# NilFoundation/crypto3-zk

Hardware: AMD Instinct MI355X
Metric: MSM Mpoints/sec, BLS12-381 G1 Pippenger, 2^20 points per GPU (higher is better)
Workload: dtype u32; 1 GPU; BLS12-381 G1 Pippenger MSM, ONE MSM of 1 x 2^20 random points/scalars, bases resident; points_per_gpu=1048576, parallelism=point-range partition x1 + one all-gather of the 144-B partial sums

## Files before the change

crypto3-zk_amd/csrc/curve.hpp:

```cpp
#pragma once
#include "fu.hpp"
#include "glv.hpp"

namespace zkhip {

template <class F>
struct Affine {
    F x, y;
    ZK_HD bool is_inf() const { return FieldOps<F>::is_exact_zero(x) && FieldOps<F>::is_exact_zero(y); }
    ZK_HD static Affine infinity() { return {F::zero(), F::zero()}; }
};

template <class F>
struct XYZZ {
    F X, Y, ZZ, ZZZ;
    ZK_HD bool is_inf() const { return FieldOps<F>::is_exact_zero(ZZ); }
    ZK_HD static XYZZ infinity() { return {F::zero(), F::zero(), F::zero(), F::zero()}; }
    ZK_HD static XYZZ from_affine(const Affine<F> &p) {
        if (p.is_inf()) return infinity();
        return {p.x, p.y, F::one(), F::one()};
    }
};

template <class F>
struct Jacobian {
    F X, Y, Z;
};

template <class F>
ZK_HD XYZZ<F> xyzz_dbl_affine(const Affine<F> &p) {
    typedef FieldOps<F> O;
    if (p.is_inf()) return XYZZ<F>::infinity();
    F U = O::add(p.y, p.y);
    F V = O::sqr(U);
    F W = O::mul(U, V);
    F S = O::mul(p.x, V);
    F xx = O::sqr(p.x);
    F M = O::add(O::add(xx, xx), xx);
    F X3 = O::template sub<O::K1>(O::sqr(M), O::add(S, S));
    F Y3 = O::template mul_sub<O::K2>(M, O::template sub<O::K2>(S, X3), W, p.y);
    return {X3, Y3, V, W};
}

template <class F>
ZK_HD XYZZ<F> xyzz_dbl(const XYZZ<F> &a) {
    typedef FieldOps<F> O;
    if (a.is_inf()) return XYZZ<F>::infinity();
    F U = O::add(a.Y, a.Y);
    F V = O::sqr(U);
    F W = O::mul(U, V);
    F S = O::mul(a.X, V);
    F xx = O::sqr(a.X);
    F M = O::add(O::add(xx, xx), xx);
    F X3 = O::template sub<O::K1>(O::sqr(M), O::add(S, S));
    F Y3 = O::template mul_sub<O::K2>(M, O::template sub<O::K2>(S, X3), W, a.Y);
    return {X3, Y3, O::mul(V, a.ZZ), O::mul(W, a.ZZZ)};
}

template <class F>
ZK_HD XYZZ<F> xyzz_madd(const XYZZ<F> &a, const Affine<F> &p_in, bool negate = false) {
    typedef FieldOps<F> O;
    if (p_in.is_inf()) return a;
    Affine<F> p = p_in;
    if (negate) p.y = O::template sub<O::K1>(F::zero(), p.y);
    if (a.is_inf()) return {p.x, p.y, F::one(), F::one()};
    F U2 = O::mul(p.x, a.ZZ);
    F S2 = O::mul(p.y, a.ZZZ);
    F Pd = O::template sub<O::K2>(U2, a.X);
    F R = O::template sub<O::K2>(S2, a.Y);
    F PP = O::sqr(Pd);
    if (O::is_zero_product(PP)) {
        if (O::is_zero(R)) return xyzz_dbl_affine(p);
        return XYZZ<F>::infinity();
    }
    F PPP = O::mul(Pd, PP);
    F Q = O::mul(a.X, PP);
    F X3 = O::template sub<O::K1>(O::sqr(R), O::add(PPP, O::add(Q, Q)));
    F Y3 = O::template mul_sub<O::K2>(R, O::template sub<O::K2>(Q, X3), a.Y, PPP);
    return {X3, Y3, O::mul(a.ZZ, PP), O::mul(a.ZZZ, PPP)};
}

template <class F>
ZK_HD XYZZ<F> xyzz_add(const XYZZ<F> &a, const XYZZ<F> &b) {
    typedef FieldOps<F> O;
    if (a.is_inf()) return b;
    if (b.is_inf()) return a;
    F U1 = O::mul(a.X, b.ZZ);
    F U2 = O::mul(b.X, a.ZZ);
    F S1 = O::mul(a.Y, b.ZZZ);
    F S2 = O::mul(b.Y, a.ZZZ);
    F Pd = O::template sub<O::K1>(U2, U1);
    F R = O::template sub<O::K1>(S2, S1);
    F PP = O::sqr(Pd);
    if (O::is_zero_product(PP)) {
        if (O::is_zero(R)) return xyzz_dbl(a);
        return XYZZ<F>::infinity();
    }
    F PPP = O::mul(Pd, PP);
    F Q = O::mul(U1, PP);
    F X3 = O::template sub<O::K1>(O::sqr(R), O::add(PPP, O::add(Q, Q)));
    F Y3 = O::template mul_sub<O::K1>(R, O::template sub<O::K2>(Q, X3), S1, PPP);
    return {X3, Y3, O::mul(O::mul(a.ZZ, b.ZZ), PP), O::mul(O::mul(a.ZZZ, b.ZZZ), PPP)};
}

template <class F>
ZK_HD XYZZ<F> xyzz_mul_small(const XYZZ<F> &a, uint32_t k) {
    XYZZ<F> r = XYZZ<F>::infinity();
    if (k == 0 || a.is_inf()) return r;
    int top = 31;
    while (!((k >> top) & 1)) --top;
    if (top == 0) return a;
    const XYZZ<F> a2 = xyzz_dbl(a), a3 = xyzz_add(a2, a);
    for (int i = top >> 1; i >= 0; --i) {
        if (!r.is_inf()) r = xyzz_dbl(xyzz_dbl(r));
        const uint32_t d = (k >> (2 * i)) & 3u;
        if (d != 0) r = xyzz_add(r, d == 1 ? a : (d == 2 ? a2 : a3));
    }
    return r;
}

template <class F>
ZK_HD Jacobian<F> xyzz_to_jacobian(const XYZZ<F> &a) {
    typedef FieldOps<F> O;
    if (a.is_inf()) return {F::one(), F::one(), F::zero()};
    F z2 = O::sqr(a.ZZ);
    F z3 = O::sqr(a.ZZZ);
    return {O::mul(a.X, O::sqr(z2)), O::mul(a.Y, O::sqr(z3)), O::mul(a.ZZ, a.ZZZ)};
}

template <class F>
ZK_HD XYZZ<F> xyzz_from_jacobian(const Jacobian<F> &j) {
    typedef FieldOps<F> O;
    if (O::is_zero(j.Z)) return XYZZ<F>::infinity();
    F zz = O::sqr(j.Z);
    return {j.X, j.Y, zz, O::mul(zz, j.Z)};
}

template <class F>
ZK_HD Affine<F> xyzz_to_affine(const XYZZ<F> &a) {
    typedef FieldOps<F> O;
    if (a.is_inf()) return Affine<F>::infinity();
    F i = O::inv(O::mul(a.ZZ, a.ZZZ));
    return {O::mul(a.X, O::mul(i, a.ZZZ)), O::mul(a.Y, O::mul(i, a.ZZ))};
}

template <class F>
ZK_HD Affine<F> affine_load(const uint32_t *p) {
    typedef FieldOps<F> O;
    return {O::load(p), O::load(p + O::WORDS)};
}
template <class F>
ZK_HD void affine_store(uint32_t *p, const Affine<F> &a) {
    typedef FieldOps<F> O;
    O::store(p, a.x);
    O::store(p + O::WORDS, a.y);
}
template <class F>
ZK_HD XYZZ<F> xyzz_load(const uint32_t *p) {
    typedef FieldOps<F> O;
    constexpr int W = O::WORDS;
    return {O::load(p), O::load(p + W), O::load(p + 2 * W), O::load(p + 3 * W)};
}
template <class F>
ZK_HD void xyzz_store(uint32_t *p, const XYZZ<F> &a) {
    typedef FieldOps<F> O;
    constexpr int W = O::WORDS;
    O::store(p, a.X);
    O::store(p + W, a.Y);
    O::store(p + 2 * W, a.ZZ);
    O::store(p + 3 * W, a.ZZZ);
}

template <class F>
ZK_HD void xyzz_store_canonical_jacobian(uint32_t *dst, const XYZZ<F> &p) {
    constexpr int CW = FieldOps<F>::CANON_WORDS;
    Jacobian<F> j = xyzz_to_jacobian(p);
    FieldOps<F>::to_canonical(dst, j.X);
    FieldOps<F>::to_canonical(dst + CW, j.Y);
    FieldOps<F>::to_canonical(dst + 2 * CW, j.Z);
}

template <class F>
ZK_HD void xyzz_park(uint32_t *pt, uint32_t *pre_slot, const XYZZ<F> &q, F &pre) {
    typedef FieldOps<F> O;
    xyzz_store<F>(pt, q);
    if (!q.is_inf()) pre = O::mul(pre, O::mul(q.ZZ, q.ZZZ));
    O::store(pre_slot, pre);
}
template <class F, class Pt, class Pre, class Out>
ZK_HD void xyzz_parked_to_affine(const F &pre_all, uint32_t cnt, Pt pt, Pre pre, Out out) {
    typedef FieldOps<F> O;
    F inv = O::inv(pre_all);
    for (uint32_t k = cnt; k-- > 0;) {
        XYZZ<F> q = xyzz_load<F>(pt(k));
        if (q.is_inf()) {
            affine_store<F>(out(k), Affine<F>::infinity());
            continue;
        }
        F before = k > 0 ? O::load(pre(k - 1)) : F::one();
        F dinv = O::mul(inv, before);
        inv = O::mul(inv, O::mul(q.ZZ, q.ZZZ));
        Affine<F> a = {O::mul(q.X, O::mul(dinv, q.ZZZ)), O::mul(q.Y, O::mul(dinv, q.ZZ))};
        affine_store<F>(out(k), a);
    }
}
constexpr uint32_t AFFINE_MAX_CHUNK = 8;
inline uint32_t affine_chunk(size_t points) {
    uint32_t chunk = 1;
    while (chunk < AFFINE_MAX_CHUNK && (points + chunk - 1) / chunk > 16384) chunk <<= 1;
    return chunk;
}

template <int CURVE, int GROUP>
struct CurveTraits;
template <>
struct CurveTraits<CURVE_BLS12_381, GROUP_G1> {
    typedef bls_fqu F;
};
template <>
struct CurveTraits<CURVE_BLS12_381, GROUP_G2> {
    typedef bls_fqu2 F;
};
template <>
struct CurveTraits<CURVE_BN254, GROUP_G1> {
    typedef bn_fqu F;
};
template <>
struct CurveTraits<CURVE_BN254, GROUP_G2> {
    typedef bn_fqu2 F;
};
template <>
struct CurveTraits<CURVE_PALLAS, GROUP_G1> {
    typedef pallas_fqu F;
};
template <>
// ... 27 lines not shown
```

crypto3-zk_amd/csrc/msm_bucket_acc.hpp:

```cpp
#pragma once
#include "curve.hpp"
#include "fu2_pair.hpp"

namespace zkhip {

template <class F>
struct LimbView;
template <class U>
struct LimbView<Fu<U>> {
    static constexpr int N = U::L;
    ZK_D static uint32_t get(const Fu<U> &x, int i) { return x.v[i]; }
    ZK_D static void set(Fu<U> &x, int i, uint32_t v) { x.v[i] = v; }
};
template <class U>
struct LimbView<Fu2h<U>> {
    static constexpr int N = U::L;
    ZK_D static uint32_t get(const Fu2h<U> &x, int i) { return x.v.v[i]; }
    ZK_D static void set(Fu2h<U> &x, int i, uint32_t v) { x.v.v[i] = v; }
};

template <class F, int NT>
struct LdsAcc {
    typedef LimbView<F> V;
    static constexpr int Q = (V::N + 3) / 4;
    static constexpr size_t BYTES = (size_t)3 * Q * NT * 16;
    uint4 *base;
    uint32_t t;
    ZK_D F get(int coord) const {
        uint32_t w[4 * Q];
#pragma unroll
        for (int q = 0; q < Q; ++q) {
            uint4 v = base[(coord * Q + q) * NT + t];
            w[4 * q] = v.x, w[4 * q + 1] = v.y, w[4 * q + 2] = v.z, w[4 * q + 3] = v.w;
        }
        F r;
#pragma unroll
        for (int i = 0; i < V::N; ++i) V::set(r, i, w[i]);
        return r;
    }
    ZK_D void put(int coord, const F &x) const {
#pragma unroll
        for (int q = 0; q < Q; ++q) {
            uint4 v;
            v.x = 4 * q + 0 < V::N ? V::get(x, 4 * q + 0) : 0u;
            v.y = 4 * q + 1 < V::N ? V::get(x, 4 * q + 1) : 0u;
            v.z = 4 * q + 2 < V::N ? V::get(x, 4 * q + 2) : 0u;
            v.w = 4 * q + 3 < V::N ? V::get(x, 4 * q + 3) : 0u;
            base[(coord * Q + q) * NT + t] = v;
        }
    }
};

template <class F, int NT, int WAVES, int LPB = 1>
__global__ __launch_bounds__(NT, WAVES) void msm_bucket_acc_lds(const uint32_t *__restrict__ bases, const uint32_t *__restrict__ offs,
                                                           const uint32_t *__restrict__ idx, uint32_t nbuckets, uint32_t large,
                                                           const uint32_t *__restrict__ order, uint32_t *__restrict__ buckets) {
    typedef FieldOps<F> O;
    constexpr int NL = O::WORDS;
    extern __shared__ __attribute__((aligned(16))) uint4 acc_lds[];
    const uint32_t tid = threadIdx.x, slot = (blockIdx.x * NT + tid) / LPB;
    if (slot >= nbuckets) return;
    const uint32_t g = order[slot];
    const uint32_t lo = offs[g], hi = offs[g + 1];
    if (hi - lo > large) return;
    LdsAcc<F, NT> A = {acc_lds, tid};
    enum { CX = 0, CY = 1, CZZ = 2 };
    F ZZZ = F::zero();
    bool inf = true;
    for (uint32_t k = lo; k < hi; ++k) {
        const uint32_t e = idx[k];
        Affine<F> p = affine_load<F>(bases + (size_t)(e & 0x7FFFFFFFu) * (2 * NL));
        if (p.is_inf()) continue;
        if (e >> 31) p.y = O::template sub<O::K1>(F::zero(), p.y);
        if (inf) {
            A.put(CX, p.x);
            A.put(CY, p.y);
            A.put(CZZ, F::one());
            ZZZ = F::one();
            inf = false;
            continue;
        }
        F Pd = O::template sub<O::K2>(O::mul(p.x, A.get(CZZ)), A.get(CX));
        F R = O::template sub<O::K2>(O::mul(p.y, ZZZ), A.get(CY));
        F PP = O::sqr(Pd);
        if (O::is_zero_product(PP)) {
            if (O::is_zero(R)) {
                XYZZ<F> d = xyzz_dbl_affine(p);
                A.put(CX, d.X);
                A.put(CY, d.Y);
                A.put(CZZ, d.ZZ);
                ZZZ = d.ZZZ;
            } else {
                inf = true;
            }
            continue;
        }
        F PPP = O::mul(Pd, PP);
        F Q = O::mul(A.get(CX), PP);
        F X3 = O::template sub<O::K1>(O::sqr(R), O::add(PPP, O::add(Q, Q)));
        F Y3 = O::template mul_sub<O::K2>(R, O::template sub<O::K2>(Q, X3), A.get(CY), PPP);
        A.put(CX, X3);
        A.put(CY, Y3);
        A.put(CZZ, O::mul(A.get(CZZ), PP));
        ZZZ = O::mul(ZZZ, PPP);
    }
    XYZZ<F> out = XYZZ<F>::infinity();
    if (!inf) out = {A.get(CX), A.get(CY), A.get(CZZ), ZZZ};
    xyzz_store<F>(buckets + (size_t)g * (4 * NL), out);
}

}
```

crypto3-zk_amd/csrc/msm_core.hpp:

```cpp
#pragma once
#include <algorithm>
#include <string>
#include <type_traits>
#include <vector>

#ifndef ZK_NOINLINE_MUL2
#define ZK_NOINLINE_MUL2 1
#endif
#include "ctx.hpp"
#include "curve.hpp"
#include "msm_entries.hpp"
#include "msm_ops.hpp"
#include "msm_recode.hpp"
#include "msm_bucket_acc.hpp"
#include "fu_pair.hpp"
#include "fu_quad.hpp"
#include "fu_wide.hpp"

namespace {

using namespace zkhip;

#ifndef MSM_G1_THREADS
#define MSM_G1_THREADS 64
// ... 42 lines not shown
    const uint32_t nlarge = plan[1], t = threadIdx.x / LPB;
    for (uint32_t j = blockIdx.x; j < nlarge; j += gridDim.x) {
        const uint32_t g = large[3 * j], first = large[3 * j + 1], nt = large[3 * j + 2];
        XYZZ<F> acc = XYZZ<F>::infinity();
        for (uint32_t k = t; k < nt; k += 64 / LPB) acc = xyzz_add(acc, xyzz_load<F>(partials + (size_t)(first + k) * (4 * NL)));
        if (nt > 1) {
            xyzz_store<F>(lds + (size_t)t * (4 * NL), acc);
            __syncthreads();
            for (uint32_t d = 32 / LPB; d >= 1; d >>= 1) {
                if (t < d && t + d < nt) {
                    acc = xyzz_add(xyzz_load<F>(lds + (size_t)t * (4 * NL)), xyzz_load<F>(lds + (size_t)(t + d) * (4 * NL)));
                    xyzz_store<F>(lds + (size_t)t * (4 * NL), acc);
                }
                __syncthreads();
            }
        }
        if (t == 0) xyzz_store<F>(buckets + (size_t)g * (4 * NL), acc);
        __syncthreads();
    }
}

template <class F, int LPB>
__global__ __launch_bounds__(256) void msm_bucket_merge(uint32_t *__restrict__ buckets, uint32_t B, uint32_t q, uint32_t cur) {
    constexpr int NL = FieldOps<F>::WORDS;
    uint32_t g = (blockIdx.x * blockDim.x + threadIdx.x) / LPB;
    if (g >= q * B) return;
    const uint32_t s = g / B;
    uint32_t *dst = buckets + (size_t)g * (4 * NL);
    XYZZ<F> acc = xyzz_load<F>(dst);
    for (uint32_t k = 1; k < 4; ++k)
        if (s + k * q < cur) acc = xyzz_add(acc, xyzz_load<F>(buckets + ((size_t)g + (size_t)k * q * B) * (4 * NL)));
    xyzz_store<F>(dst, acc);
}

constexpr int MSM_TAIL_THREADS = 256;

template <class F>
ZK_D XYZZ<F> block_tree_sum(uint32_t *lds, XYZZ<F> acc, uint32_t t, uint32_t nthreads) {
    constexpr int NL = FieldOps<F>::WORDS;
    xyzz_store<F>(lds + (size_t)t * (4 * NL), acc);
    __syncthreads();
    for (uint32_t d = nthreads / 2; d >= 1; d >>= 1) {
        if (t < d) {
            acc = xyzz_add(xyzz_load<F>(lds + (size_t)t * (4 * NL)), xyzz_load<F>(lds + (size_t)(t + d) * (4 * NL)));
            xyzz_store<F>(lds + (size_t)t * (4 * NL), acc);
        }
        __syncthreads();
    }
    return acc;
}

template <class F, int LPB>
#ifndef ZK_TAIL_WAVES
#define ZK_TAIL_WAVES 2
#endif
__global__ __launch_bounds__(MSM_TAIL_THREADS, ZK_TAIL_WAVES) void msm_bucket_red(const uint32_t *__restrict__ buckets, uint32_t B, uint32_t L, uint32_t nseg,
                                                                   uint32_t nblk, uint32_t *__restrict__ partial) {
    constexpr int NL = FieldOps<F>::WORDS;
    extern __shared__ __attribute__((aligned(16))) uint32_t lds[];
    constexpr uint32_t SLOTS = MSM_TAIL_THREADS / LPB;
    const uint32_t t = threadIdx.x / LPB, w = blockIdx.x / nblk, seg = (blockIdx.x % nblk) * SLOTS + t;
    XYZZ<F> sum = XYZZ<F>::infinity();
    if (seg < nseg) {
        const uint32_t *base = buckets + ((size_t)w * B + (size_t)seg * L) * (4 * NL);
        if (L == 1) {
            sum = xyzz_mul_small(xyzz_load<F>(base), seg + 1);
        } else {
            XYZZ<F> run = XYZZ<F>::infinity();
            for (int b = (int)L - 1; b >= 0; --b) {
                run = xyzz_add(run, xyzz_load<F>(base + (size_t)b * (4 * NL)));
                sum = xyzz_add(sum, run);
            }
            if (seg != 0) sum = xyzz_add(sum, xyzz_mul_small(run, seg * L));
        }
    }
    sum = block_tree_sum<F>(lds, sum, t, SLOTS);
    if (t == 0) xyzz_store<F>(partial + (size_t)blockIdx.x * (4 * NL), sum);
}

template <class F, int LPB>
__global__ __launch_bounds__(256) void msm_window_sum(const uint32_t *__restrict__ partial, uint32_t nblk, uint32_t *__restrict__ winsum) {
    constexpr int NL = FieldOps<F>::WORDS;
    extern __shared__ __attribute__((aligned(16))) uint32_t lds[];
    const uint32_t w = blockIdx.x, t = threadIdx.x / LPB, slots = blockDim.x / LPB;
    XYZZ<F> acc = XYZZ<F>::infinity();
    for (uint32_t j = t; j < nblk; j += slots) acc = xyzz_add(acc, xyzz_load<F>(partial + ((size_t)w * nblk + j) * (4 * NL)));
    if (nblk > 1) acc = block_tree_sum<F>(lds, acc, t, slots);
    if (t == 0) xyzz_store<F>(winsum + (size_t)w * (4 * NL), acc);
}
inline uint32_t msm_window_threads(uint32_t nblk, int lanes_per_point) { return (size_t)nblk * lanes_per_point > 128 ? 256u : 64u; }

struct MsmFold {
    uint32_t B, C, R, log_c;
    uint32_t run;
    uint32_t m_row, m_col;
};
inline MsmFold msm_fold_geom(const zkhip_ctx *ctx, uint32_t B) {
    MsmFold g;
    int lb = 0;
    while ((1u << lb) < B) ++lb;
    g.B = B;
    g.log_c = (uint32_t)((lb + 1) / 2);
    g.C = 1u << g.log_c;
    g.R = B >> g.log_c;
    g.run = ctx->opt_msm_fold_run > 0 ? (uint32_t)ctx->opt_msm_fold_run : (B >= (1u << 18) ? 8u : 4u);
    g.run = std::max(1u, std::min(g.run, g.R));
    g.m_row = g.C / g.run;
    g.m_col = g.R / g.run;
    return g;
}

template <class FA, int LA, class FT, int LT>
__global__ __launch_bounds__(MSM_TAIL_THREADS, ZK_TAIL_WAVES) void msm_fold(const uint32_t *__restrict__ buckets, MsmFold g, uint32_t *__restrict__ level2) {
    constexpr int NL = FieldOps<FA>::WORDS;
    constexpr uint32_t SA = MSM_TAIL_THREADS / LA, ST = MSM_TAIL_THREADS / LT, PW = 4 * NL;
    extern __shared__ __attribute__((aligned(16))) uint32_t lds[];
    const uint32_t half_wgs = g.B / (SA * g.run);
    const uint32_t w = blockIdx.x / (2 * half_wgs), k = blockIdx.x % (2 * half_wgs);
    const bool col = k >= half_wgs;
    const uint32_t wg = col ? k - half_wgs : k, s = threadIdx.x / LA;
    const uint32_t m = col ? g.m_col : g.m_row, G = SA / m;
    uint32_t first, stride, slot;
    if (!col) {
        first = (wg * G + s / m) * g.C + s % m;
        stride = m;
        slot = s;
    } else {
        const uint32_t j = s / G, ll = s % G;
        first = j * g.C + wg * G + ll;
        stride = m * g.C;
        slot = ll * m + j;
    }
    {
        const uint32_t *src = buckets + ((size_t)w * g.B + first) * PW;
        XYZZ<FA> acc = xyzz_load<FA>(src);
        for (uint32_t i = 1; i < g.run; ++i) acc = xyzz_add(acc, xyzz_load<FA>(src + (size_t)i * stride * PW));
        xyzz_store<FA>(lds + (size_t)slot * PW, acc);
    }
    __syncthreads();
    const uint32_t t = threadIdx.x / LT;
    for (uint32_t half = m / 2; half >= 1; half >>= 1) {
        const uint32_t adds = G * half;
        for (uint32_t idx = t; idx < adds; idx += ST) {
            uint32_t *p = lds + (size_t)((idx / half) * m + idx % half) * PW;
            xyzz_store<FT>(p, xyzz_add(xyzz_load<FT>(p), xyzz_load<FT>(p + (size_t)half * PW)));
        }
        __syncthreads();
    }
    for (uint32_t i = t; i < G; i += ST) {
        const uint32_t o = wg * G + i;
        if (col || o != 0)
            xyzz_store<FT>(level2 + (((size_t)2 * w + (col ? 0 : 1)) * g.C + (col ? o : o - 1)) * PW, xyzz_load<FT>(lds + (size_t)i * m * PW));
    }
}

template <class F, int LPB>
__global__ __launch_bounds__(64) void msm_final_fold(const uint32_t *__restrict__ winsum, uint32_t count, uint32_t shift, uint32_t *const *__restrict__ outs,
                                                     uint32_t *__restrict__ out) {
    constexpr int NL = FieldOps<F>::WORDS;
    if (blockIdx.x >= count || threadIdx.x >= LPB) return;
    XYZZ<F> acc = xyzz_load<F>(winsum + ((size_t)2 * blockIdx.x + 1) * (4 * NL));
    if (!acc.is_inf())
        for (uint32_t i = 0; i < shift; ++i) acc = xyzz_dbl(acc);
    acc = xyzz_add(acc, xyzz_load<F>(winsum + (size_t)2 * blockIdx.x * (4 * NL)));
    xyzz_store_canonical_jacobian<F>(outs ? outs[blockIdx.x] : out, acc);
}

constexpr uint32_t MSM_WIDE_WAVES = 8;

template <class U>
ZK_D XYZZ<FuW<U>> wide_tree_sum(uint32_t *lds, XYZZ<FuW<U>> acc, uint32_t w, uint32_t nw) {
    constexpr uint32_t PW = 4 * U::SL;
    wide_store<U>(lds + w * PW, acc);
    __syncthreads();
    for (uint32_t d = nw / 2; d >= 1; d >>= 1) {
        if (w < d) {
            acc = xyzz_add(wide_load<U>(lds + w * PW), wide_load<U>(lds + (w + d) * PW));
            wide_store<U>(lds + w * PW, acc);
        }
        __syncthreads();
    }
    return acc;
}

template <class U>
__global__ __launch_bounds__(MSM_WIDE_WAVES * 64) void msm_wide_weigh(const uint32_t *__restrict__ points, uint32_t C, uint32_t *__restrict__ partial) {
    constexpr uint32_t PW = 4 * U::SL;
    __shared__ uint32_t lds[MSM_WIDE_WAVES * PW];
    const uint32_t w = threadIdx.x >> 6, i = blockIdx.x * MSM_WIDE_WAVES + w;
    XYZZ<FuW<U>> acc = xyzz_mul_small(wide_load<U>(points + (size_t)i * PW), (i & (C - 1)) + 1);
    acc = wide_tree_sum<U>(lds, acc, w, MSM_WIDE_WAVES);
    if (w == 0) wide_store<U>(partial + (size_t)blockIdx.x * PW, acc);
}

template <class U>
__global__ __launch_bounds__(MSM_WIDE_WAVES * 64) void msm_wide_tree(const uint32_t *__restrict__ in, uint32_t *__restrict__ out) {
    constexpr uint32_t PW = 4 * U::SL;
    __shared__ uint32_t lds[MSM_WIDE_WAVES * PW];
    const uint32_t w = threadIdx.x >> 6;
    const uint32_t *src = in + ((size_t)blockIdx.x * 2 * MSM_WIDE_WAVES + w) * PW;
    XYZZ<FuW<U>> acc = xyzz_add(wide_load<U>(src), wide_load<U>(src + (size_t)MSM_WIDE_WAVES * PW));
    acc = wide_tree_sum<U>(lds, acc, w, MSM_WIDE_WAVES);
    if (w == 0) wide_store<U>(out + (size_t)blockIdx.x * PW, acc);
}

template <class U>
__global__ __launch_bounds__(MSM_WIDE_WAVES * 64) void msm_wide_final(const uint32_t *__restrict__ partial, uint32_t m, uint32_t shift, uint32_t *const *__restrict__ outs,
                                                                      uint32_t *__restrict__ out) {
    constexpr uint32_t PW = 4 * U::SL, HALF = MSM_WIDE_WAVES / 2;
    __shared__ uint32_t lds[MSM_WIDE_WAVES * PW];
    const uint32_t w = threadIdx.x >> 6, half = w / HALF, q = w % HALF;
    const uint32_t *src = partial + ((size_t)2 * blockIdx.x + (1 - half)) * m * PW;
    XYZZ<FuW<U>> acc = XYZZ<FuW<U>>::infinity();
    for (uint32_t j = q; j < m; j += HALF) acc = xyzz_add(acc, wide_load<U>(src + (size_t)j * PW));
    acc = wide_tree_sum<U>(lds + half * HALF * PW, acc, q, HALF);
    if (w != 0) return;
    if (!acc.is_inf())
        for (uint32_t i = 0; i < shift; ++i) acc = xyzz_dbl(acc);
    acc = xyzz_add(acc, wide_load<U>(lds + HALF * PW));
    const XYZZ<FuQ<U>> whole = wide_gather<U>(acc);
    if (wide_lane() < 4) xyzz_store_canonical_jacobian<FuQ<U>>(outs ? outs[blockIdx.x] : out, whole);
}

template <class F, int LPB>
__global__ __launch_bounds__(64) void msm_final(const uint32_t *__restrict__ winsum, int W, MsmWindows win, uint32_t *__restrict__ out_jac) {
    constexpr int NL = FieldOps<F>::WORDS;
    if (blockIdx.x != 0 || threadIdx.x >= LPB) return;
    XYZZ<F> acc = XYZZ<F>::infinity();
    for (int w = W - 1; w >= 0; --w) {
        if (!acc.is_inf())
            for (int i = 0; i < win.width(w); ++i) acc = xyzz_dbl(acc);
        acc = xyzz_add(acc, xyzz_load<F>(winsum + (size_t)w * (4 * NL)));
    }
    xyzz_store_canonical_jacobian<F>(out_jac, acc);
}

template <class F>
__global__ __launch_bounds__(256) void bases_to_mont(const uint32_t *__restrict__ canon, const uint8_t *__restrict__ inf, uint32_t n,
                                                     uint32_t *__restrict__ pts) {
    typedef FieldOps<F> O;
    uint32_t i = blockIdx.x * blockDim.x + threadIdx.x;
    if (i >= n) return;
    const uint32_t *c = canon + (size_t)i * (2 * O::CANON_WORDS);
    Affine<F> a;
    if (inf != nullptr && inf[i]) a = Affine<F>::infinity();
    else a = {O::from_canonical(c), O::from_canonical(c + O::CANON_WORDS)};
    affine_store<F>(pts + (size_t)i * (2 * O::WORDS), a);
}

template <class F>
__global__ __launch_bounds__(256) void bases_from_mont(const uint32_t *__restrict__ pts, uint32_t n, uint32_t *__restrict__ out,
                                                       uint8_t *__restrict__ inf) {
    typedef FieldOps<F> O;
    uint32_t i = blockIdx.x * blockDim.x + threadIdx.x;
    if (i >= n) return;
    Affine<F> a = affine_load<F>(pts + (size_t)i * (2 * O::WORDS));
    inf[i] = a.is_inf() ? 1 : 0;
    uint32_t *o = out + (size_t)i * (2 * O::CANON_WORDS);
    O::to_canonical(o, a.x);
    O::to_canonical(o + O::CANON_WORDS, a.y);
}

template <class F>
__global__ __launch_bounds__(64) void bases_mul(uint32_t *__restrict__ pts, const uint32_t *__restrict__ base_canonical,
                                                const uint32_t *__restrict__ scalars, uint32_t n) {
    constexpr int NL = FieldOps<F>::WORDS;
    uint32_t i = blockIdx.x * blockDim.x + threadIdx.x;
    if (i >= n) return;
    Affine<F> g = {FieldOps<F>::from_canonical(base_canonical), FieldOps<F>::from_canonical(base_canonical + FieldOps<F>::CANON_WORDS)};
    const uint32_t *s = scalars + (size_t)i * 8;
    XYZZ<F> acc = XYZZ<F>::infinity();
    for (int b = 255; b >= 0; --b) {
        acc = xyzz_dbl(acc);
        if ((s[b >> 5] >> (b & 31)) & 1) acc = xyzz_madd(acc, g);
    }
    affine_store<F>(pts + (size_t)i * (2 * NL), xyzz_to_affine(acc));
}

constexpr int FIXED_WBITS = 8, FIXED_NW = 32, FIXED_ROW = 1 << FIXED_WBITS;
template <class F>
__global__ __launch_bounds__(64) void bases_fixed_table(const uint32_t *__restrict__ base_canonical, uint32_t *__restrict__ tab, uint32_t *__restrict__ tmp) {
    typedef FieldOps<F> O;
    constexpr int NL = O::WORDS;
    const uint32_t w = blockIdx.x * blockDim.x + threadIdx.x;
    if (w >= FIXED_NW) return;
    Affine<F> g = {O::from_canonical(base_canonical), O::from_canonical(base_canonical + O::CANON_WORDS)};
    XYZZ<F> P = XYZZ<F>::from_affine(g);
    for (uint32_t k = 0; k < w * FIXED_WBITS; ++k) P = xyzz_dbl(P);
    uint32_t *mine = tmp + (size_t)w * FIXED_ROW * (5 * NL);
    XYZZ<F> acc = P;
    F pre = F::one();
    for (uint32_t d = 1; d < FIXED_ROW; ++d) {
        if (d > 1) acc = xyzz_add(acc, P);
        uint32_t *slot = mine + (size_t)d * (5 * NL);
        xyzz_store<F>(slot, acc);
        pre = O::mul(pre, O::mul(acc.ZZ, acc.ZZZ));
        O::store(slot + 4 * NL, pre);
    }
    F inv = O::inv(pre);
    for (uint32_t d = FIXED_ROW; d-- > 1;) {
        const uint32_t *slot = mine + (size_t)d * (5 * NL);
        XYZZ<F> q = xyzz_load<F>(slot);
        F before = d > 1 ? O::load(mine + (size_t)(d - 1) * (5 * NL) + 4 * NL) : F::one();
        F dinv = O::mul(inv, before);
        inv = O::mul(inv, O::mul(q.ZZ, q.ZZZ));
        Affine<F> a = {O::mul(q.X, O::mul(dinv, q.ZZZ)), O::mul(q.Y, O::mul(dinv, q.ZZ))};
// ... 93 lines not shown
    O::to_canonical(aff + CW, a.y);
}

template <class F>
__global__ void jac_sum_k(const uint32_t *__restrict__ jac, uint32_t count, uint32_t *__restrict__ out) {
    typedef FieldOps<F> O;
    constexpr int CW = O::CANON_WORDS;
    if (blockIdx.x != 0 || threadIdx.x != 0) return;
    XYZZ<F> acc = XYZZ<F>::infinity();
    for (uint32_t i = 0; i < count; ++i) {
        const uint32_t *p = jac + (size_t)i * 3 * CW;
        Jacobian<F> j = {O::from_canonical(p), O::from_canonical(p + CW), O::from_canonical(p + 2 * CW)};
        acc = xyzz_add(acc, xyzz_from_jacobian(j));
    }
    Jacobian<F> r = xyzz_to_jacobian(acc);
    O::to_canonical(out, r.X);
    O::to_canonical(out + CW, r.Y);
    O::to_canonical(out + 2 * CW, r.Z);
}

template <class F>
__global__ void msm_write_infinity(uint32_t *out_jac) {
    if (blockIdx.x != 0 || threadIdx.x != 0) return;
    xyzz_store_canonical_jacobian<F>(out_jac, XYZZ<F>::infinity());
}

template <class F, int LPB>
__global__ __launch_bounds__(64) void msm_final_batch(const uint32_t *__restrict__ winsum, uint32_t count, uint32_t *const *__restrict__ outs) {
    constexpr int NL = FieldOps<F>::WORDS;
    constexpr int CW = FieldOps<F>::CANON_WORDS;
    if (blockIdx.x >= count || threadIdx.x >= LPB) return;
    Jacobian<F> j = xyzz_to_jacobian(xyzz_load<F>(winsum + (size_t)blockIdx.x * (4 * NL)));
    uint32_t *out = outs[blockIdx.x];
    FieldOps<F>::to_canonical(out, j.X);
    FieldOps<F>::to_canonical(out + CW, j.Y);
    FieldOps<F>::to_canonical(out + 2 * CW, j.Z);
}


inline uint32_t msm_tail_segment(const zkhip_ctx *ctx, uint32_t B, size_t sets, int lanes_per_point) {
    uint32_t L = 1;
    if (ctx->opt_msm_segment_log >= 0) L = 1u << std::min(ctx->opt_msm_segment_log, 8);
    else {
        const size_t lanes = sets * B * (size_t)lanes_per_point;
        while (L < 16 && lanes / L > 65536) L <<= 1;
        while (L < 64 && lanes / L > 262144) L <<= 1;
    }
    return std::min(B, L);
}

struct MsmTailGeom {
    uint32_t L, nseg;
    uint32_t slots, nblk;
    uint32_t wthreads;
    size_t lds_red, lds_win;
};
template <class Lane>
MsmTailGeom msm_tail_geom(const zkhip_ctx *ctx, uint32_t B, size_t sets) {
    constexpr size_t point_bytes = (size_t)4 * FieldOps<typename Lane::type>::WORDS * 4;
    constexpr int XL = Lane::LANES;
    MsmTailGeom t;
    t.L = msm_tail_segment(ctx, B, sets, XL);
    t.nseg = B / t.L;
    t.slots = MSM_TAIL_THREADS / XL;
    t.nblk = (t.nseg + t.slots - 1) / t.slots;
    t.wthreads = msm_window_threads(t.nblk, XL);
    t.lds_red = t.slots * point_bytes;
    t.lds_win = t.wthreads / XL * point_bytes;
    return t;
}

template <class Lane, class Final>
int msm_tail(zkhip_ctx *ctx, const uint32_t *sets, size_t nsets, uint32_t B, uint32_t *segsum, size_t segsum_blocks, uint32_t *winsum, Final final) {
    typedef typename Lane::type TX;
    constexpr int XL = Lane::LANES;
    const MsmTailGeom t = msm_tail_geom<Lane>(ctx, B, nsets);
    if (nsets * t.nblk > segsum_blocks) {
        ctx->last_error = "MSM tail of " + std::to_string(nsets * t.nblk) + " workgroups over a partial-sum buffer for " + std::to_string(segsum_blocks);
        return ZKHIP_ERR_RANGE;
    }
    ZK_MAX_LDS(ctx, (msm_bucket_red<TX, XL>), t.lds_red);
    ZK_LAUNCH(ctx, "msm_bucket_red", (msm_bucket_red<TX, XL>), dim3((unsigned)(nsets * t.nblk)), dim3(MSM_TAIL_THREADS), t.lds_red, sets, B, t.L, t.nseg, t.nblk,
              segsum);
    ZK_LAUNCH(ctx, "msm_window_sum", (msm_window_sum<TX, XL>), dim3((unsigned)nsets), dim3(t.wthreads), t.lds_win, segsum, t.nblk, winsum);
    return final();
}

template <class F>
bool msm_fold_applies(const zkhip_ctx *ctx, uint32_t B, bool tables) {
    if (FieldOps<F>::WORDS > 16 && !ctx->opt_msm_tail_fold_g2) return false;
    if (!tables || ctx->opt_msm_tail_fold <= 0 || B < (1u << std::min(ctx->opt_msm_tail_fold, 30))) return false;
    const MsmFold g = msm_fold_geom(ctx, B);
    const uint32_t sa = MSM_TAIL_THREADS / BucketLane<F>::LANES;
    return g.m_col >= 1 && g.m_row <= sa && g.m_col <= sa && B >= sa * g.run && g.m_row * g.run == g.C && g.m_col * g.run == g.R;
}
template <class F>
struct MsmFoldBuffers {
    static constexpr size_t PW = (size_t)4 * FieldOps<F>::WORDS;
    MsmFold g{};
    size_t nsets = 0;
    uint32_t *level2 = nullptr, *segsum = nullptr, *winsum = nullptr;
    MsmFoldBuffers() = default;
    MsmFoldBuffers(const zkhip_ctx *ctx, uint32_t B, size_t nsets_) : g(msm_fold_geom(ctx, B)), nsets(nsets_) {}
    size_t level2_words() const { return nsets * 2 * g.C * PW; }
    size_t segsum_blocks() const { return nsets * 2 * std::max<size_t>((g.C + 63) / 64, WideLane<F>::AVAILABLE && nsets == 1 ? g.C / MSM_WIDE_WAVES : 0); }
    template <class Arena>
    void layout(Arena &a) {
        a.take(level2, level2_words());
        a.take(segsum, segsum_blocks() * PW);
        a.take(winsum, nsets * 2 * PW);
    }
};

template <class F>
bool msm_tail_wide_applies(const zkhip_ctx *ctx, size_t nsets, uint32_t C) {
    return WideLane<F>::AVAILABLE && ctx->opt_msm_tail_quads == 1 && nsets == 1 && C >= MSM_WIDE_WAVES;
}
template <class F>
int msm_tail_wide(zkhip_ctx *ctx, const MsmFoldBuffers<F> &fb, uint32_t *const *d_outs, uint32_t *d_out) {
    if constexpr (WideLane<F>::AVAILABLE) {
        typedef typename F::params U;
        const uint32_t C = fb.g.C;
        const size_t sets = 2 * fb.nsets;
        uint32_t m = C / MSM_WIDE_WAVES;
        if (sets * m > fb.segsum_blocks()) {
            ctx->last_error = "wide MSM tail of " + std::to_string(sets * m) + " workgroups over a partial-sum buffer for " + std::to_string(fb.segsum_blocks());
            return ZKHIP_ERR_RANGE;
        }
        uint32_t *from = fb.segsum, *to = fb.level2;
        ZK_LAUNCH(ctx, "msm_wide_weigh", (msm_wide_weigh<U>), dim3((unsigned)(sets * m)), dim3(MSM_WIDE_WAVES * 64), 0, fb.level2, C, from);
        while (m > MSM_WIDE_WAVES) {
            m /= 2 * MSM_WIDE_WAVES;
            ZK_LAUNCH(ctx, "msm_wide_tree", (msm_wide_tree<U>), dim3((unsigned)(sets * m)), dim3(MSM_WIDE_WAVES * 64), 0, from, to);
            std::swap(from, to);
        }
        ZK_LAUNCH(ctx, "msm_wide_final", (msm_wide_final<U>), dim3((unsigned)fb.nsets), dim3(MSM_WIDE_WAVES * 64), 0, from, m, fb.g.log_c, d_outs, d_out);
        return 0;
    } else {
        (void)fb, (void)d_outs, (void)d_out;
        ctx->last_error = "no wide lane for this field";
        return ZKHIP_ERR_INVALID;
    }
}

template <class F, class Lane>
int msm_fold_tail(zkhip_ctx *ctx, const uint32_t *sets, const MsmFoldBuffers<F> &fb, uint32_t *const *d_outs, uint32_t *d_out) {
    constexpr int NL = FieldOps<F>::WORDS;
    typedef typename BucketLane<F>::type FL;
    constexpr int LPB = BucketLane<F>::LANES;
    typedef typename QuadLane<F>::type TQ;
    constexpr int QL = QuadLane<F>::LANES;
    const MsmFold &g = fb.g;
    const size_t nsets = fb.nsets;
    ZK_HIP_CHECK(ctx, hipMemsetAsync(fb.level2, 0, fb.level2_words() * 4, ctx->stream));
    const size_t lds = (size_t)MSM_TAIL_THREADS / LPB * 4 * NL * 4;
    ZK_MAX_LDS(ctx, (msm_fold<FL, LPB, TQ, QL>), lds);
    ZK_LAUNCH(ctx, "msm_fold", (msm_fold<FL, LPB, TQ, QL>), dim3((unsigned)(nsets * (g.B / (MSM_TAIL_THREADS / LPB * g.run)) * 2)), dim3(MSM_TAIL_THREADS), lds,
              sets, g, fb.level2);
    auto level2 = [&](auto lane) -> int {
        typedef decltype(lane) X;
        return msm_tail<X>(ctx, fb.level2, 2 * nsets, g.C, fb.segsum, fb.segsum_blocks(), fb.winsum, [&]() -> int {
            ZK_LAUNCH(ctx, "msm_final", (msm_final_fold<typename X::type, X::LANES>), dim3((unsigned)nsets), dim3(64), 0, fb.winsum, (uint32_t)nsets, g.log_c, d_outs, d_out);
            return 0;
        });
    };
    if (msm_tail_wide_applies<F>(ctx, nsets, g.C)) return msm_tail_wide<F>(ctx, fb, d_outs, d_out);
    if (QuadLane<F>::AVAILABLE && ctx->opt_msm_tail_quads && 2 * nsets * g.C <= ((size_t)1 << 18)) return level2(QuadLane<F>());
    return level2(Lane());
}

struct MsmCall : MsmEntriesCall {
    int Sr;
    uint32_t segsum_blocks;
    bool fold;
};

template <class F>
int msm_call_plan(const zkhip_ctx *ctx, const zkhip_bases *bases, size_t offset, size_t n, bool batch_member, MsmCall &c, std::string &error) {
    ZK_TRY(zk_msm_entries_plan(ctx, bases, offset, n, c, error));
    const MsmPlan &P = c.P;
    c.Sr = P.tables ? 1 : P.W;
    c.segsum_blocks = std::max(msm_tail_geom<TailLane<F>>(ctx, P.B, c.Sr).nblk, msm_tail_geom<QuadLane<F>>(ctx, P.B, c.Sr).nblk);
    c.fold = !batch_member && msm_fold_applies<F>(ctx, P.B, P.tables);
    return 0;
}

template <class F>
struct MsmBuffers : MsmEntriesBuffers {
    static constexpr size_t PW = (size_t)4 * FieldOps<F>::WORDS;
    const MsmCall &c;
    uint32_t *buckets;
    uint32_t *segsum, *winsum;
    MsmFoldBuffers<F> fb;
    uint32_t *partials;
    MsmBuffers(const zkhip_ctx *ctx, const MsmCall &call) : c(call) {
        if (c.fold) fb = MsmFoldBuffers<F>(ctx, c.P.B, 1);
    }
    template <class Arena>
    void layout(Arena &a) {
        a.take(dig, c.entries());
        a.take(bh, c.nbh);
        a.take(bo, (size_t)c.nbh + 1);
        a.take(bsums, (c.nbh + 1023) / 1024);
        a.take(tmp_idx, c.entries());
        a.take(tmp_key, c.entries());
        a.take(offs, (size_t)c.P.nb + 1);
        a.take(idx, c.entries());
        a.take(buckets, c.P.nb * PW);
        a.take(sh, (size_t)c.nsh + 1);
        a.take(so, (size_t)c.nsh + 1);
        a.take(ssums, (c.nsh + 1023) / 1024);
        a.take(order, c.P.nb);
        a.take(segsum, (size_t)c.Sr * c.segsum_blocks * PW);
        a.take(winsum, (size_t)std::max(1, c.Sr) * PW);
        if (c.fold) fb.layout(a);
        a.take(plan, 4);
        a.take(tasks, (size_t)c.task_cap * 3);
        a.take(large, (size_t)c.large_cap * 3);
        a.take(partials, c.task_cap * PW);
    }
};

template <class F>
int msm_stages(zkhip_ctx *ctx, const zkhip_bases *bases, const MsmCall &c, const MsmBuffers<F> &w, const uint32_t *d_scalars, bool reuse_sort) {
    constexpr int NL = FieldOps<F>::WORDS;
    typedef typename BucketLane<F>::type FL;
    constexpr int LPB = BucketLane<F>::LANES;
    const MsmPlan &P = c.P;
    const uint32_t nb = P.nb;
    const uint32_t *d_b = bases->d;
    if (!reuse_sort) ZK_TRY(zk_msm_entries(ctx, bases->curve, c, w, d_scalars));
    if constexpr (FieldOps<F>::WORDS <= 16) {
        constexpr int NT = MSM_G1_THREADS;
        size_t lds_acc = LdsAcc<F, NT>::BYTES;
        ZK_MAX_LDS(ctx, (msm_bucket_acc_lds<F, NT, 3>), lds_acc);
        ZK_LAUNCH(ctx, "msm_bucket_acc", (msm_bucket_acc_lds<F, NT, 3>), dim3((nb + NT - 1) / NT), dim3(NT), lds_acc, d_b, w.offs, w.idx, nb, c.large_thresh,
                  w.order, w.buckets);
    } else {
        constexpr int NT = MSM_G2_THREADS, WAVES = MSM_G2_WAVES;
        size_t lds_acc = LdsAcc<FL, NT>::BYTES;
        ZK_MAX_LDS(ctx, (msm_bucket_acc_lds<FL, NT, WAVES, LPB>), lds_acc);
        ZK_LAUNCH(ctx, "msm_bucket_acc", (msm_bucket_acc_lds<FL, NT, WAVES, LPB>), dim3((unsigned)(((size_t)nb * LPB + NT - 1) / NT)), dim3(NT), lds_acc, d_b,
                  w.offs, w.idx, nb, c.large_thresh, w.order, w.buckets);
    }
    if (!reuse_sort) ZK_TRY(zk_msm_large_plan(ctx, c, w));
    {
        size_t lds_large = (size_t)128 / LPB * 4 * NL * 4;
        if (lds_large > 48 * 1024) ZK_MAX_LDS(ctx, (msm_bucket_large<FL, LPB>), lds_large);
        unsigned grid_large = (unsigned)std::min<size_t>(c.task_cap, 512);
        ZK_LAUNCH(ctx, "msm_bucket_large", (msm_bucket_large<FL, LPB>), dim3(grid_large), dim3(128), lds_large, d_b, w.idx, w.plan, w.tasks, w.partials);
        ZK_LAUNCH(ctx, "msm_bucket_large", (msm_large_combine<FL, LPB>), dim3((unsigned)std::min<uint32_t>(c.large_cap, 256)), dim3(64),
                  (size_t)64 / LPB * 4 * NL * 4, w.plan, w.large, w.partials, w.buckets);
    }
    if (P.tables) {
        for (uint32_t cur = P.S; cur > 1;) {
            const uint32_t q = (cur + 3) / 4;
            ZK_LAUNCH(ctx, "msm_bucket_merge", (msm_bucket_merge<FL, LPB>), grid_1d((size_t)q * P.B * LPB), dim3(256), 0, w.buckets, P.B, q,
                      cur);
            cur = q;
        }
    }
    return 0;
}

template <class F>
int msm_run_t(zkhip_ctx *ctx, const zkhip_bases *bases, size_t offset, size_t n, const uint32_t *d_scalars, uint32_t *d_out_jac) {
    MsmCall c;
    ZK_TRY(msm_call_plan<F>(ctx, bases, offset, n, false, c, ctx->last_error));
    MsmBuffers<F> w(ctx, c);
    ZK_TRY(ws_place(ctx, w));
    ZK_TRY(msm_stages<F>(ctx, bases, c, w, d_scalars, false));
    if (c.fold) return msm_fold_tail<F, TailLane<F>>(ctx, w.buckets, w.fb, nullptr, d_out_jac);
    auto tail = [&](auto lane) -> int {
        typedef decltype(lane) X;
        return msm_tail<X>(ctx, w.buckets, (size_t)c.Sr, c.P.B, w.segsum, (size_t)c.Sr * c.segsum_blocks, w.winsum, [&]() -> int {
            ZK_LAUNCH(ctx, "msm_final", (msm_final<typename X::type, X::LANES>), dim3(1), dim3(64), 0, w.winsum, c.Sr, c.P.win, d_out_jac);
            return 0;
        });
    };
    if (QuadLane<F>::AVAILABLE && ctx->opt_msm_tail_quads && (size_t)c.Sr * c.P.B <= ((size_t)1 << 18)) return tail(QuadLane<F>());
    return tail(TailLane<F>());
}

template <class F>
int msm_batch_member(zkhip_ctx *ctx, const zkhip_bases *bases, size_t offset, size_t n, const uint32_t *d_scalars, uint32_t *slot, bool reuse_sort) {
    MsmCall c;
    ZK_TRY(msm_call_plan<F>(ctx, bases, offset, n, true, c, ctx->last_error));
    MsmBuffers<F> w(ctx, c);
    ZK_TRY(ws_place(ctx, w));
    if (c.P.S == 1) w.buckets = slot;
    ZK_TRY(msm_stages<F>(ctx, bases, c, w, d_scalars, reuse_sort));
    if (w.buckets != slot) ZK_HIP_CHECK(ctx, hipMemcpyAsync(slot, w.buckets, c.P.B * MsmBuffers<F>::PW * 4, hipMemcpyDeviceToDevice, ctx->stream));
    return 0;
}

struct BasesTmp {
    size_t words;
    uint32_t *tmp;
    template <class Arena>
    void layout(Arena &a) { a.take(tmp, words); }
};

template <class F>
int bases_precompute_t(zkhip_ctx *ctx, zkhip_bases *b) {
    constexpr int NL = FieldOps<F>::WORDS;
    if (!b->tables() || b->n == 0) return 0;
    const size_t chunk = 1u << 18;
// ... 156 lines not shown
```

Baseline: 437.6 Mpoints/s.

## Skip ZZ/ZZZ multiplies on fresh bucket, prefetch indices, zero level2 tail in-kernel

In the single-lane bucket accumulator, the first addition after loading an affine point is now treated as affine+affine, which skips four field multiplies for that step. The next bucket index is also loaded one iteration ahead. The separate memset of the level2 buffer is dropped; the fold kernel instead zeroes only the unused tail entries of the odd column. The goal is fewer multiplies per bucket and one less full-buffer memset, at the cost of extra control flow and relying on the fold kernel to write every level2 slot that is later read. An unused xyzz_add_affine helper is also added.

```diff
diff --git a/crypto3-zk_amd/csrc/curve.hpp b/crypto3-zk_amd/csrc/curve.hpp
--- a/crypto3-zk_amd/csrc/curve.hpp
+++ b/crypto3-zk_amd/csrc/curve.hpp
@@ -81,6 +81,25 @@
 }
 
 template <class F>
+ZK_HD XYZZ<F> xyzz_add_affine(const Affine<F> &a, const Affine<F> &b) {
+    typedef FieldOps<F> O;
+    if (b.is_inf()) return XYZZ<F>::from_affine(a);
+    if (a.is_inf()) return XYZZ<F>::from_affine(b);
+    F Pd = O::template sub<O::K2>(b.x, a.x);
+    F R = O::template sub<O::K2>(b.y, a.y);
+    F PP = O::sqr(Pd);
+    if (O::is_zero_product(PP)) {
+        if (O::is_zero(R)) return xyzz_dbl_affine(b);
+        return XYZZ<F>::infinity();
+    }
+    F PPP = O::mul(Pd, PP);
+    F Q = O::mul(a.x, PP);
+    F X3 = O::template sub<O::K1>(O::sqr(R), O::add(PPP, O::add(Q, Q)));
+    F Y3 = O::template mul_sub<O::K2>(R, O::template sub<O::K2>(Q, X3), a.y, PPP);
+    return {X3, Y3, PP, PPP};
+}
+
+template <class F>
 ZK_HD XYZZ<F> xyzz_add(const XYZZ<F> &a, const XYZZ<F> &b) {
     typedef FieldOps<F> O;
     if (a.is_inf()) return b;
diff --git a/crypto3-zk_amd/csrc/msm_bucket_acc.hpp b/crypto3-zk_amd/csrc/msm_bucket_acc.hpp
--- a/crypto3-zk_amd/csrc/msm_bucket_acc.hpp
+++ b/crypto3-zk_amd/csrc/msm_bucket_acc.hpp
@@ -67,21 +67,30 @@
     enum { CX = 0, CY = 1, CZZ = 2 };
     F ZZZ = F::zero();
     bool inf = true;
+    bool fresh = false;
+    uint32_t e_next = lo < hi ? idx[lo] : 0u;
     for (uint32_t k = lo; k < hi; ++k) {
-        const uint32_t e = idx[k];
+        const uint32_t e = e_next;
+        if (k + 1 < hi) e_next = idx[k + 1];
         Affine<F> p = affine_load<F>(bases + (size_t)(e & 0x7FFFFFFFu) * (2 * NL));
         if (p.is_inf()) continue;
         if (e >> 31) p.y = O::template sub<O::K1>(F::zero(), p.y);
         if (inf) {
             A.put(CX, p.x);
             A.put(CY, p.y);
-            A.put(CZZ, F::one());
+            if (LPB != 1) A.put(CZZ, F::one());
             ZZZ = F::one();
             inf = false;
+            fresh = LPB == 1;
             continue;
         }
-        F Pd = O::template sub<O::K2>(O::mul(p.x, A.get(CZZ)), A.get(CX));
-        F R = O::template sub<O::K2>(O::mul(p.y, ZZZ), A.get(CY));
+        F Pd = p.x, R = p.y;
+        if (!fresh) {
+            Pd = O::mul(p.x, A.get(CZZ));
+            R = O::mul(p.y, ZZZ);
+        }
+        Pd = O::template sub<O::K2>(Pd, A.get(CX));
+        R = O::template sub<O::K2>(R, A.get(CY));
         F PP = O::sqr(Pd);
         if (O::is_zero_product(PP)) {
             if (O::is_zero(R)) {
@@ -93,6 +102,7 @@
             } else {
                 inf = true;
             }
+            fresh = false;
             continue;
         }
         F PPP = O::mul(Pd, PP);
@@ -101,11 +111,17 @@
         F Y3 = O::template mul_sub<O::K2>(R, O::template sub<O::K2>(Q, X3), A.get(CY), PPP);
         A.put(CX, X3);
         A.put(CY, Y3);
-        A.put(CZZ, O::mul(A.get(CZZ), PP));
-        ZZZ = O::mul(ZZZ, PPP);
+        if (fresh) {
+            A.put(CZZ, PP);
+            ZZZ = PPP;
+            fresh = false;
+        } else {
+            A.put(CZZ, O::mul(A.get(CZZ), PP));
+            ZZZ = O::mul(ZZZ, PPP);
+        }
     }
     XYZZ<F> out = XYZZ<F>::infinity();
-    if (!inf) out = {A.get(CX), A.get(CY), A.get(CZZ), ZZZ};
+    if (!inf) out = {A.get(CX), A.get(CY), fresh ? F::one() : A.get(CZZ), ZZZ};
     xyzz_store<F>(buckets + (size_t)g * (4 * NL), out);
 }
 
diff --git a/crypto3-zk_amd/csrc/msm_core.hpp b/crypto3-zk_amd/csrc/msm_core.hpp
--- a/crypto3-zk_amd/csrc/msm_core.hpp
+++ b/crypto3-zk_amd/csrc/msm_core.hpp
@@ -218,6 +218,12 @@
         if (col || o != 0)
             xyzz_store<FT>(level2 + (((size_t)2 * w + (col ? 0 : 1)) * g.C + (col ? o : o - 1)) * PW, xyzz_load<FT>(lds + (size_t)i * m * PW));
     }
+    if (!col) {
+        for (uint32_t e = g.R - 1 + wg; e < g.C; e += half_wgs) {
+            uint32_t *z = level2 + (((size_t)2 * w + 1) * g.C + e) * PW;
+            for (uint32_t i = threadIdx.x; i < PW; i += MSM_TAIL_THREADS) z[i] = 0u;
+        }
+    }
 }
 
 template <class F, int LPB>
@@ -617,7 +623,6 @@
     constexpr int QL = QuadLane<F>::LANES;
     const MsmFold &g = fb.g;
     const size_t nsets = fb.nsets;
-    ZK_HIP_CHECK(ctx, hipMemsetAsync(fb.level2, 0, fb.level2_words() * 4, ctx->stream));
     const size_t lds = (size_t)MSM_TAIL_THREADS / LPB * 4 * NL * 4;
     ZK_MAX_LDS(ctx, (msm_fold<FL, LPB, TQ, QL>), lds);
     ZK_LAUNCH(ctx, "msm_fold", (msm_fold<FL, LPB, TQ, QL>), dim3((unsigned)(nsets * (g.B / (MSM_TAIL_THREADS / LPB * g.run)) * 2)), dim3(MSM_TAIL_THREADS), lds,
```

Result: faster. 447.8 Mpoints/s (median of 6 runs) (+2.3%).
